# terra-render/Terra

Hardware: AMD Instinct MI355X
Metric: Msamples/s (higher is better)
Workload: dtype f32; 1 GPU; cornell_1080p_512spp; scene=cornell32, width=1920, height=1080, spp=512, bounces=8, integrator=simple, triangles=32, tree=auto, traversal=reference tree + leaf-box cull, tile=64, sample_split=8, parallelism=single

## Files before the change

include/terra_amd.h:

```cpp
#ifndef TERRA_AMD_H
#define TERRA_AMD_H

#include "Terra.h"

#ifdef __cplusplus
extern "C" {
#endif

typedef enum {
    kTerraAmdOk               = 0,
    kTerraAmdErrNoDevice      = -1,
    kTerraAmdErrNotCommitted  = -2,
    kTerraAmdErrUnsupported   = -3,
    kTerraAmdErrBadArgument   = -4,
    kTerraAmdErrLaunch        = -5
} TerraAmdStatus;

const char* terra_amd_last_error ( void );
void        terra_amd_clear_error ( void );
int         terra_amd_first_error ( char* buf, size_t capacity );
void        terra_amd_clear_first_error ( void );
size_t      terra_amd_thread_staging_bytes ( void );

int  terra_amd_init ( void );
// ... 65 lines not shown
int  terra_amd_set_job_order ( HTerraScene scene, int on );
int  terra_amd_get_job_order ( HTerraScene scene );

int  terra_amd_set_empty_skip ( HTerraScene scene, int on );
int  terra_amd_get_empty_skip ( HTerraScene scene );
int  terra_amd_empty_skip_info ( HTerraScene scene, uint32_t out[2] );
int  terra_amd_empty_proof ( const float* cam_rot9, const float* cam_pos3, float tan_half_fov, float aspect, float jitter, uint32_t fb_w, uint32_t fb_h,
                             uint32_t x0, uint32_t y0, uint32_t x1, uint32_t y1, const float* tris9, size_t n_tris );

int  terra_amd_set_leaf_box_test ( HTerraScene scene, int on );
int  terra_amd_get_leaf_box_test ( HTerraScene scene );
int  terra_amd_leaf_box_info ( HTerraScene scene, uint32_t out[2] );
int  terra_amd_set_leaf_pairs ( HTerraScene scene, int on );
int  terra_amd_get_leaf_pairs ( HTerraScene scene );
int  terra_amd_leaf_pair_info ( HTerraScene scene, uint32_t out[2] );

int  terra_amd_set_environment_lighting ( HTerraScene scene, int on );
int  terra_amd_get_environment_lighting ( HTerraScene scene );

int  terra_amd_set_sampler_integration ( HTerraScene scene, int on );
int  terra_amd_get_sampler_integration ( HTerraScene scene );

int  terra_amd_set_environment_sampling ( HTerraScene scene, int on );
int  terra_amd_get_environment_sampling ( HTerraScene scene );

int  terra_amd_set_environment_mis ( HTerraScene scene, int on );
int  terra_amd_get_environment_mis ( HTerraScene scene );

int terra_amd_set_work_counters ( HTerraScene scene, int on );
int terra_amd_get_work_counters ( HTerraScene scene );
// ... 296 lines not shown
```

terra_amd/csrc/dev_types.h:

```cpp
#pragma once
#include <stdint.h>
#include <stddef.h>
#include <hip/hip_vector_types.h>

#define TERRA_DEV_MAX_ATTR 8

struct DevF3 { float x, y, z; };
struct DevF4 { float x, y, z, w; };

#define DEV_CHILD_LEAF  0x80000000u
#define DEV_CHILD_EMPTY 0xFFFFFFFFu

struct DevNode {
    float    min0[3], max0[3];
    float    min1[3], max1[3];
    uint32_t child[2];
    uint32_t prim[2];
};
static_assert ( sizeof ( DevNode ) == 64, "DevNode must be 64 bytes" );

struct DevFastNode {
    uint32_t q[3][2][4];
    uint32_t child[4];
    uint32_t pad[4];
// ... 68 lines not shown
struct DevLeafPair { uint32_t tri[2]; uint32_t rank[2]; };
static_assert ( sizeof ( DevLeafPair ) == 16, "DevLeafPair must be 16 bytes" );
constexpr uint32_t terra_leaf_pair_words_entry_of ( uint32_t n_tris ) { return 2u * n_tris; }
constexpr uint32_t terra_leaf_pair_words_masks ( uint32_t n_tris ) { return 3u * n_tris; }
#define TERRA_PAIR_ENTRY_BYTES 64
#define TERRA_PAIR_BOX_STRIDE 48
constexpr uint32_t terra_pair_entry_offset ( uint32_t n_pairs, uint32_t perm, uint32_t e ) { return TERRA_PAIR_ENTRY_BYTES * ( perm * n_pairs + e ); }
constexpr uint32_t terra_pair_boxes_offset ( uint32_t n_pairs ) { return 6u * TERRA_PAIR_ENTRY_BYTES * n_pairs; }
constexpr uint32_t terra_pair_box_plane_offset ( uint32_t k, uint32_t a, uint32_t s ) { return TERRA_PAIR_BOX_STRIDE * k + 8u * ( 2u * a + s ); }
constexpr uint32_t terra_pair_section_bytes ( uint32_t n_pairs ) { return terra_pair_boxes_offset ( n_pairs ) + TERRA_PAIR_BOX_STRIDE * n_pairs; }
static_assert ( terra_pair_box_plane_offset ( 7, 0, 0 ) == 336 && terra_pair_box_plane_offset ( 0, 2, 1 ) + 8u == TERRA_PAIR_BOX_STRIDE, "a box = six 8-byte plane pairs; a group of eight within 384 bytes" );
#define TERRA_SHADE_CONSTS_BYTES 48u
static_assert ( terra_pair_section_bytes ( TERRA_LEAF_RANK_MAX / 2 ) + TERRA_SHADE_CONSTS_BYTES * TERRA_LEAF_RANK_MAX <= 6u * TERRA_RANKED_ENTRY_BYTES * TERRA_LEAF_RANK_MAX
                && terra_pair_section_bytes ( 1 ) + TERRA_SHADE_CONSTS_BYTES * 2u <= 6u * TERRA_RANKED_ENTRY_BYTES * 2u, "pair section + shading constants fit where the plan budgeted ranked entries" );
static_assert ( terra_pair_section_bytes ( TERRA_LEAF_RANK_MAX / 2 ) <= 6u * TERRA_RANKED_ENTRY_BYTES * TERRA_LEAF_RANK_MAX && terra_pair_section_bytes ( 1 ) <= 6u * TERRA_RANKED_ENTRY_BYTES * 2u, "the pair section never takes more LDS than the ranked entries it replaces" );
constexpr uint32_t terra_pair_key ( uint32_t rank, uint32_t tri ) { return ( rank + 1u ) << 5 | tri; }
static_assert ( TERRA_LEAF_RANK_MAX <= 32, "a pair key keeps the triangle in five bits" );
#define TERRA_LEAF_CAP_MAX 16
#define TERRA_COL 256
#define TERRA_LDS_NODE_BYTES 112
#define TERRA_AUX_WORDS 6
#define TERRA_AUX_WORDS_LDS 9
#ifndef TERRA_FAST_STACK_LDS
#define TERRA_FAST_STACK_LDS 16
#endif
#ifndef TERRA_LDS_CU_KB
#define TERRA_LDS_CU_KB 158
#endif
#ifndef TERRA_LEAF_CAP_MIN
#define TERRA_LEAF_CAP_MIN 6
// ... 119 lines not shown
```

terra_amd/csrc/render_kernels.hip:

```cpp
#include <hip/hip_runtime.h>
#include "trace_device.h"
#include "kernels.h"
#include "launch_plan.h"
#include "empty_proof.h"

#ifdef TERRA_TU
#define TERRA_TU_HAS(k) ( TERRA_TU == ( k ) )
#define TERRA_TU_MODE(k) ( TERRA_TU == ( k ) || TERRA_TU == ( k ) + 4 || TERRA_TU == ( k ) + 8 || TERRA_TU == ( k ) + 12 )
#else
#define TERRA_TU_HAS(k) ( !TERRA_RAY_SOURCE )
#define TERRA_TU_MODE(k) 1
#endif
#if TERRA_RAY_SOURCE == 3
typedef DevPointRenderParams RenderKernelParams;
#elif TERRA_RAY_SOURCE == 2
typedef DevLensRenderParams RenderKernelParams;
#elif TERRA_RAY_SOURCE == 1
typedef DevRayRenderParams RenderKernelParams;
#else
typedef DevRenderParams RenderKernelParams;
#endif

struct DevResult { float acc[3]; int samples; };

// ... 1 lines not shown
    const uint32_t v[6] = { c.rays, c.nodes, c.tri_tests, c.hits, c.rand_calls, c.attr_fetches };
    const int slot[6] = { kCtrRays, kCtrNodes, kCtrTriTests, kCtrHits, kCtrRandCalls, kCtrAttrFetches };
    #pragma unroll
    for ( int k = 0; k < 6; ++k ) {
        unsigned long long x = v[k];
        #pragma unroll
        for ( int off = 32; off > 0; off >>= 1 ) x += __shfl_xor ( x, off, 64 );
        if ( ( threadIdx.x & 63 ) == 0 && x ) atomicAdd ( &g[slot[k]], x );
    }
}

#ifndef TERRA_CHECK_SHRINK
#define TERRA_CHECK_SHRINK 0
#endif
TD const uint32_t* terra_leaf_pair_table ( const DevRenderParams& p ) {
    return p.leaf_pairs ? reinterpret_cast<const uint32_t*> ( reinterpret_cast<const char*> ( p.scene.tris ) + p.leaf_pairs ) : nullptr;
}
template <int MODE>
TD Tracer make_tracer ( const DevScene& sc, float4* lds, uint32_t stack_depth, uint32_t leaf_cap, uint32_t lds_nodes, uint32_t lds_tris, bool cull, bool fused, bool ranked,
                        const DevLeafBox* leaf_boxes, uint32_t n_leaf_boxes, const uint32_t* leaf_pairs ) {
    const int tid = threadIdx.x;
    Tracer T;
    T.sc = sc;
    float4* ln = lds;
    float4* lt = ln + ( TERRA_LDS_NODE_BYTES / 16 ) * lds_nodes;
    float4* lp = lt + 3 * lds_tris;
    uint32_t* lm = reinterpret_cast<uint32_t*> ( lp + 4 * lds_tris );
    const uint32_t m_words = MODE == 1 ? ( ( sc.n_objects * ( uint32_t ) ( sizeof ( DevMaterial ) / 4 ) + 3u ) & ~3u ) : 0u, l_words = MODE == 1 ? sc.n_lights * 4u : 0u, a_words = MODE == 1 ? ( ( sc.n_tris + 3u ) & ~3u ) : 0u;
    uint32_t* ll = lm + m_words; uint32_t* la = ll + l_words;
    ranked = MODE == 1 && ranked;
    float4* lr = reinterpret_cast<float4*> ( la + a_words );
// ... 382 lines not shown
        if ( point_inactive ( r.o, r.d ) ) j.s = p.chunk_spp;
        if ( TERRA_POINT_HOLD ) held = r;
#else
        if ( ray_record_inactive ( r ) ) j.s = p.chunk_spp;
        if ( TERRA_RAY_HOLD ) held = r;
#endif
    }
}
#endif

template <int INTEGRATOR, int COUNT, int MODE, int KINDS>
__global__ __launch_bounds__ ( 256, terra_waves ( INTEGRATOR, KINDS, MODE ) ) void terra_render_kernel ( RenderKernelParams p ) {
    extern __shared__ float4 lds_f4[];
    const int tid = threadIdx.x;
    Tracer T0 = make_tracer<MODE> ( p.scene, lds_f4, p.stack_depth, p.leaf_cap, p.lds_nodes, p.lds_tris, p.leaf_cull != 0, p.fused_slab != 0, p.leaf_rank != 0, p.leaf_boxes, p.n_leaf_boxes, terra_leaf_pair_table ( p ) );
    T0.faults = p.counters + kCtrFaults;
    if ( MODE >= 2 && p.stack_spill ) { T0.spill = p.stack_spill + ( size_t ) ( blockIdx.x * 256u + threadIdx.x ) * p.spill_cap; T0.spill_cap = p.spill_cap; }
    const Tracer T = T0;

    PixelStreams rs = trng_pixel_streams ( 0, 0, 0 );
    Counters c = counters_zero();
    float* acc_lds = reinterpret_cast<float*> ( T.stack - tid ) + ( p.stack_depth + p.leaf_cap ) * TERRA_COL + tid;
    uint32_t job_total = p.job_blocks * 256u;
    if constexpr ( MODE == 1 ) { if ( p.job_live ) job_total = *p.job_live; }
    job_init_lane ( p, acc_lds );
    Jobs jb; jb.px = jb.py = 0; jb.s = p.chunk_spp; jb.exhausted = false; jb.base = 0;
    SamplerPair sp = sampler_pair_none();
    V3 Lo = v3 ( 0, 0, 0 ), throughput = v3 ( 1, 1, 1 );
    Ray ray = make_ray ( v3 ( 0, 0, 0 ), v3 ( 0, 0, 1 ) );
    uint32_t bounce = 0;
// ... 539 lines not shown
```

terra_amd/csrc/scene_host.cpp:

```cpp
#include <hip/hip_runtime.h>
#include <algorithm>
#include <cfloat>
#include <cmath>
#include <cstdarg>
#include <cstdio>
#include <cstdlib>
#include <cstring>
#include <mutex>
#include <string>
#include <unordered_set>
#include <atomic>
#include <chrono>
#include <vector>

#include "../../include/terra_amd.h"
#include "../../include/TerraPresets.h"
#include "dev_types.h"
#include "kernels.h"
#include "launch_plan.h"
#include "empty_proof.h"
#include "tree_build.h"
#include "multi_gpu.h"

static thread_local std::string g_last_error;
// ... 287 lines not shown
    std::atomic<int> last_call { 0 };
    uint32_t sample_split = 1;
    bool env_lighting = false;
    bool work_counters = false;
    bool env_sampling = false;
    bool env_mis = false;
    int job_order = 1;
    int empty_skip = 1;
    std::atomic<uint32_t> skip_last_blocks { 0 }; std::atomic<int> skip_last_device { -1 };
    int leaf_box_test = 1;
    std::vector<DevLeafBox> leaf_boxes;
    std::atomic<uint32_t> flat_last { 0 };
    int leaf_pair_form = 1;
    std::vector<uint32_t> leaf_pairs;
    std::atomic<uint32_t> pairs_last { 0 };
    bool sampler_integration = false;
    std::string commit_error;
    std::atomic<bool> warned_camera { false };
    int test_pad_stack = 0;
    int test_fast_stack_lds = 0;
    float test_shrink_reference_boxes = 0.f;
};

static Scene* S ( HTerraScene h ) { return ( Scene* ) h; }
static const Scene::Replica& primary ( const Scene* s ) { static const Scene::Replica none; return s->replicas.empty() ? none : s->replicas[0]; }
static std::vector<int> devices_of ( const Scene* s ) { std::vector<int> d; for ( const Scene::Replica& r : s->replicas ) d.push_back ( r.device ); return d; }

static std::atomic<bool> g_commit_timing { false };
static bool timing_on() { return g_commit_timing.load ( std::memory_order_relaxed ); }
bool terra_commit_timing_on() { return timing_on(); }
// ... 117 lines not shown
extern "C" int terra_amd_set_empty_skip ( HTerraScene h, int on ) {
    if ( on < 0 || on > 1 ) return fail ( kTerraAmdErrBadArgument, "terra_amd_set_empty_skip: 0 (off) or 1 (on)" );
    S ( h )->empty_skip = on; return 0;
}
extern "C" int terra_amd_get_empty_skip ( HTerraScene h ) { return S ( h )->empty_skip; }
extern "C" int terra_amd_set_leaf_box_test ( HTerraScene h, int on ) {
    if ( on < 0 || on > 1 ) return fail ( kTerraAmdErrBadArgument, "terra_amd_set_leaf_box_test: 0 (off) or 1 (on)" );
    S ( h )->leaf_box_test = on; return 0;
}
extern "C" int terra_amd_get_leaf_box_test ( HTerraScene h ) { return S ( h )->leaf_box_test; }
extern "C" int terra_amd_set_leaf_pairs ( HTerraScene h, int on ) {
    if ( on < 0 || on > 1 ) return fail ( kTerraAmdErrBadArgument, "terra_amd_set_leaf_pairs: 0 (off) or 1 (on)" );
    S ( h )->leaf_pair_form = on; return 0;
}
extern "C" int terra_amd_get_leaf_pairs ( HTerraScene h ) { return S ( h )->leaf_pair_form; }
extern "C" int terra_amd_empty_proof ( const float* cam_rot9, const float* cam_pos3, float tan_half_fov, float aspect, float jitter, uint32_t fb_w, uint32_t fb_h,
                                       uint32_t x0, uint32_t y0, uint32_t x1, uint32_t y1, const float* tris9, size_t n_tris ) {
    if ( !cam_rot9 || !cam_pos3 || ( n_tris && !tris9 ) ) return 0;
    const TerraEmptyPlanes planes = terra_empty_planes ( cam_rot9, cam_pos3, tan_half_fov, aspect, jitter, fb_w, fb_h, x0, y0, x1, y1 );
    if ( !planes.ok ) return 0;
    for ( size_t t = 0; t < n_tris; ++t ) if ( !terra_empty_separates ( planes, tris9 + 9 * t, tris9 + 9 * t + 3, tris9 + 9 * t + 6 ) ) return 0;
    return 1;
}
extern "C" int terra_amd_set_sampler_integration ( HTerraScene h, int on ) { S ( h )->sampler_integration = on != 0; return 0; }
extern "C" int terra_amd_get_sampler_integration ( HTerraScene h ) { return S ( h )->sampler_integration ? 1 : 0; }
extern "C" void terra_amd_set_frame_seed ( HTerraScene h, uint64_t seed ) { S ( h )->frame_seed = seed; }
extern "C" uint64_t terra_amd_get_frame_seed ( HTerraScene h ) { return S ( h )->frame_seed; }

static void release_device ( Scene* s ) {
    for ( Scene::Replica& r : s->replicas ) {
// ... 160 lines not shown
    }
    if ( pairs.size() * 2 != ntri ) return none;
    std::vector<uint32_t> order ( pairs.size() );
    for ( size_t e = 0; e < order.size(); ++e ) order[e] = ( uint32_t ) e;
    auto low = [&] ( uint32_t e ) { return std::min ( pairs[e].rank[0], pairs[e].rank[1] ); };
    std::sort ( order.begin(), order.end(), [&] ( uint32_t x, uint32_t y ) { return low ( x ) < low ( y ); } );
    std::vector<uint32_t> t ( terra_leaf_pair_words_masks ( ( uint32_t ) ntri ) + boxes.size(), 0u );
    for ( size_t e = 0; e < order.size(); ++e ) {
        const DevLeafPair& p = pairs[order[e]];
        memcpy ( &t[4 * e], &p, sizeof p );
        t[terra_leaf_pair_words_entry_of ( ( uint32_t ) ntri ) + p.tri[0]] = ( uint32_t ) e; t[terra_leaf_pair_words_entry_of ( ( uint32_t ) ntri ) + p.tri[1]] = ( uint32_t ) e;
        t[terra_leaf_pair_words_masks ( ( uint32_t ) ntri ) + box_of_pair[order[e]]] |= 1u << e;
    }
    return t;
}

struct ReachTables { std::vector<DevReplay> replay; std::vector<uint32_t> leaf_parent, leaf_mask; uint64_t levels = 0, replayed = 0; };
static void build_reach_tables ( const std::vector<DevNode>& nodes, const std::vector<DevTri>& tris, const std::vector<uint32_t>& soup_of_fast, float margin, ReachTables& out ) {
    const size_t nn = nodes.size(), nt = soup_of_fast.size();
    out.replay.assign ( nn ? nn : 1, DevReplay{} );
    std::vector<uint32_t> leaf_parent_of_soup ( tris.size(), 0u );
    for ( size_t k = 0; k < nn; ++k ) for ( int c = 0; c < 2; ++c ) {
        const uint32_t w = nodes[k].child[c];
        if ( w == DEV_CHILD_EMPTY ) continue;
        if ( w & DEV_CHILD_LEAF ) { leaf_parent_of_soup[w & 0x7fffffffu] = ( uint32_t ) k; continue; }
        DevReplay& r = out.replay[w];
        memcpy ( r.bmin, c ? nodes[k].min1 : nodes[k].min0, 12 ); memcpy ( r.bmax, c ? nodes[k].max1 : nodes[k].max0, 12 );
        r.parent = ( uint32_t ) k; r.pad = 0;
    }
    auto contains = [&] ( const DevReplay & outer, const DevReplay & inner ) {
// ... 450 lines not shown
    s->tree = choose_tree ( s, f.ntri );
    TreeChoice& c = s->tree;
    if ( c.reach_cull ) for ( DevNode& d : f.nodes ) for ( int k = 0; k < 2; ++k ) {
        if ( d.child[k] == DEV_CHILD_EMPTY || ! ( d.child[k] & DEV_CHILD_LEAF ) ) continue;
        const DevTri& t = f.tris[d.child[k] & 0x7fffffffu];
        float* mn = k ? d.min1 : d.min0; float* mx = k ? d.max1 : d.max0;
        for ( int a = 0; a < 3; ++a ) {
            const float lo = std::min ( t.a[a], std::min ( t.b[a], t.c[a] ) ) - c.reach_margin, hi = std::max ( t.a[a], std::max ( t.b[a], t.c[a] ) ) + c.reach_margin;
            mn[a] = std::min ( mn[a], lo ); mx[a] = std::max ( mx[a], hi );
        }
    }
    f.leaf_boxes = leaf_box_table ( f.nodes, f.tris, f.ntri );
    s->leaf_boxes = f.leaf_boxes;
    f.leaf_pairs = leaf_pair_table ( f.leaf_boxes, f.tris, f.ntri );
    s->leaf_pairs = f.leaf_pairs;
    FastTree ft;
    if ( c.use_fast && !c.fast_on_device ) { if ( int rc = build_fast_tree_host ( s, c, f, ft ) ) return rc; }
    if ( s->tree_mode == 2 && !c.use_fast && !c.resident && f.ntri >= 2 )
        fprintf ( stderr, "[terra_amd] warning: this scene (%zu triangles) is traversed through the reference tree%s, typically 10-20 x slower than the fast tree -- %s\n", f.ntri,
                  c.cull_ok ? " with the leaf-box cull" : " decision by decision", c.note.c_str() );
    release_device ( s );
    if ( terra_amd_device_count() <= 0 ) return fail ( kTerraAmdErrNoDevice, "no HIP device visible: terra_scene_commit built the host tree but cannot upload; terra_render will fail" );
    return upload ( s, device, f, ft );
}

extern "C" void terra_scene_commit ( HTerraScene h ) {
    Scene* s = S ( h );
    const bool rebuild = s->dirty_objects || s->opts.accelerator != s->new_opts.accelerator || s->nodes.empty();
    const bool env_changed = s->env_lighting && memcmp ( &s->opts.environment_map, &s->new_opts.environment_map, sizeof ( TerraAttribute ) ) != 0;
    s->opts = s->new_opts;
// ... 214 lines not shown
    const TreeChoice& c = s->tree;
    const bool cam_ok = ray_origins_ok ? *ray_origins_ok : ( c.reach || c.reach_cull ) ? ( fabsf ( p.cam_pos[0] ) <= c.reach_limit && fabsf ( p.cam_pos[1] ) <= c.reach_limit && fabsf ( p.cam_pos[2] ) <= c.reach_limit ) : coords_within_margin ( p.cam_pos, 3 );
    if ( c.use_fast && r.dev.fast_nodes_h && ( s->tree_mode == 1 || cam_ok ) ) terra_plan_fast_tree ( p );
    else if ( ( c.use_fast || c.cull_ok ) && !cam_ok && !ray_origins_ok && !s->warned_camera.exchange ( true ) )
        fprintf ( stderr, "[terra_amd] warning: camera at (%g, %g, %g) lies outside the range (+-%g) for which this scene's traversal shortcut is proven: this call runs the reference "
                  "tree's replica traversal (same image, typically 10-20 x slower on large scenes); terra_amd_traversal_info() reports camera_limit and last_call\n",
                  ( double ) p.cam_pos[0], ( double ) p.cam_pos[1], ( double ) p.cam_pos[2], ( double ) shortcut_limit ( c ) );
    apply_stack_hooks ( s, p );
    p.leaf_cull = ( c.cull_ok && cam_ok && p.lds_mode != 2 ) ? 1u : 0u;
    p.fused_slab = ( p.leaf_cull && !c.reach_cull ) ? 1u : 0u;
    if ( s->leaf_box_test && r.d_blob && terra_leaf_boxes_fit ( p, ( uint32_t ) s->leaf_boxes.size() ) ) {
        p.leaf_boxes = ( const DevLeafBox* ) ( ( const char* ) r.d_blob + s->blob.sec[kSecLeafBoxes].offset ); p.n_leaf_boxes = ( uint32_t ) s->leaf_boxes.size();
    }
    p.leaf_pairs = 0;
    if ( s->leaf_pair_form && r.d_blob && !s->leaf_pairs.empty() && p.lds_mode == 1 && p.leaf_rank ) p.leaf_pairs = ( uint32_t ) ( s->blob.sec[kSecLeafPairs].offset - s->blob.sec[kSecTris].offset );
    if ( p.lds_mode != 1 ) p.scene.sincos24 = nullptr;
    s->last_call.store ( p.lds_mode == 2 ? ( r.dev.reach ? kTerraAmdCallFastTreeReach : kTerraAmdCallFastTree ) : ( p.leaf_cull ? kTerraAmdCallLeafCull : kTerraAmdCallReplica ), std::memory_order_relaxed );
    p.bsdf_kinds = s->bsdf_kinds;
    p.sampler_mode = 0; p.sampler_strata = ( uint32_t ) s->opts.strata;
    if ( s->sampler_integration && s->opts.sampling_method == kTerraSamplingMethodHalton ) p.sampler_mode = 1;
    if ( s->sampler_integration && s->opts.sampling_method == kTerraSamplingMethodStratified && s->opts.strata > 0 ) p.sampler_mode = 2;
    if ( p.sampler_mode ) p.bsdf_kinds |= TERRA_KIND_SAMPLER;
    if ( r.dev.env_nx && ( p.integrator == kTerraIntegratorDirect || p.integrator == kTerraIntegratorDirectMis ) ) p.bsdf_kinds |= TERRA_KIND_SAMPLER;
    else { p.scene.env_nx = 0; p.scene.env_ny = 0; }
    if ( s->env_mis && p.scene.env_nx && p.scene.env_monotone && p.integrator == kTerraIntegratorDirectMis ) p.bsdf_kinds |= TERRA_KIND_ENV_MIS;
    p.count_level = s->work_counters ? 2 : 0;
    return 0;
}

static uint64_t shard_pixels ( const DevRenderParams& p ) {
// ... 1289 lines not shown
```

terra_amd/csrc/traverse_ref.h:

```cpp
#pragma once
#include "trace_geometry.h"
#include <stddef.h>

#ifndef TERRA_PHASE_STATS
#define TERRA_PHASE_STATS 0
#endif
struct Counters {
    uint32_t rays, nodes, tri_tests, hits, rand_calls, attr_fetches;
    uint32_t tri_culled;
#if TERRA_PHASE_STATS
    uint32_t ps[16];
#endif
};
TD Counters counters_zero() {
    Counters c; c.rays = c.nodes = c.tri_tests = c.hits = c.rand_calls = c.attr_fetches = c.tri_culled = 0;
#if TERRA_PHASE_STATS
    for ( int i = 0; i < 16; ++i ) c.ps[i] = 0;
#endif
    return c;
}
#if TERRA_PHASE_STATS
#define PS_WAVE(c, k) do { if ( ( int ) ( threadIdx.x & 63 ) == __ffsll ( ( long long ) __ballot ( 1 ) ) - 1 ) ++( c ).ps[k]; } while ( 0 )
#define PS_LANE(c, k) do { ++( c ).ps[k]; } while ( 0 )
#else
// ... 17 lines not shown
    const float4* l_consts = nullptr;
    uint32_t      n_boxes;
    uint32_t      lds_nodes, lds_tris;
    int*          stack;
    int*          leaves;
    int           leaf_cap;
    int           stack_cap;
    uint32_t      stack_lim;
    uint32_t*     spill;
    uint32_t      spill_cap;
    unsigned long long* faults;
    bool cull;
    bool fused;
    bool ranked;
    bool pairs;
};
TD Tracer unstaged_tracer ( const DevScene& sc, int* words, uint32_t stack_depth, uint32_t leaf_cap, uint32_t* spill, uint32_t spill_cap ) {
    Tracer T;
    T.sc = sc; T.l_nodes = nullptr; T.l_tris = nullptr; T.l_props = nullptr; T.l_ranked = nullptr; T.n_boxes = 0;
    T.l_mats = sc.mats; T.l_lights = sc.lights; T.l_area = sc.tri_area;
    T.lds_nodes = 0; T.lds_tris = 0; T.ranked = false; T.pairs = false;
    T.stack = words + threadIdx.x; T.leaves = words + stack_depth * TERRA_COL + threadIdx.x; T.leaf_cap = ( int ) leaf_cap; T.stack_cap = ( int ) stack_depth;
    T.stack_lim = ( uint32_t ) ( uintptr_t ) words + stack_depth * 1024u;
    T.spill = spill ? spill + ( size_t ) ( blockIdx.x * 256u + threadIdx.x ) * spill_cap : nullptr; T.spill_cap = spill ? spill_cap : 0u;
    T.faults = nullptr; T.cull = false; T.fused = false;
    return T;
}

struct Closest { float depth; uint32_t tri; };

// ... 67 lines not shown

template <int COUNT, int MODE, bool ANYHIT = false>
TD void leaf_step ( const Tracer& T, const int* entry, const RayState& st, V3 o_perm, Closest& best, Counters& c, uint32_t expected = 0xffffffffu, bool* stop = nullptr ) {
    const float4* g_tris = reinterpret_cast<const float4*> ( T.sc.tris );
    PS_WAVE ( c, kPsLeafIter ); PS_LANE ( c, kPsLeafLanes );
    const uint32_t ti = ( uint32_t ) * entry;
    if ( ti == ( DEV_CHILD_EMPTY & 0x7fffffffu ) ) return;
    const TriPerm tp = MODE == 1 ? tri_perm_lds ( T.l_tris + 12 * ti, st ) : tri_perm ( g_tris[3 * ti], g_tris[3 * ti + 1], g_tris[3 * ti + 2], st );
    if ( COUNT ) ++c.tri_tests;
    float depth;
    if ( watertight_permuted ( tp, o_perm, st, depth ) && depth < best.depth ) { best.depth = depth; best.tri = ti; if ( ANYHIT && ti != expected ) *stop = true; }
}

typedef float PlanePair __attribute__ (( ext_vector_type ( 2 ) ));
typedef const __attribute__ (( address_space ( 3 ) )) PlanePair* LdsPlanes;
TD void leaf_box_test ( uint32_t bx, uint32_t by, uint32_t bz, const char* pm, const Ray& r, const SlabSel& sel, uint32_t& leaf_set, Counters& c ) {
    PS_WAVE ( c, kPsNodeIter ); PS_LANE ( c, kPsNodeLanes );
    const PlanePair ax = * ( LdsPlanes ) ( uintptr_t ) bx, ay = * ( LdsPlanes ) ( uintptr_t ) by, az = * ( LdsPlanes ) ( uintptr_t ) bz;
    const uint32_t m = *reinterpret_cast<const uint32_t*> ( pm );
    float te;
    const bool hit = slab_near_far_fused ( ax.x, ax.y, ay.x, ay.y, az.x, az.y, r, sel.oi, te );
    leaf_set |= hit ? m : 0u;
}
template <int N, uint32_t STRIDE>
TD void leaf_box_group ( uint32_t& bx, uint32_t& by, uint32_t& bz, const char*& pm, const Ray& r, const SlabSel& sel, uint32_t& leaf_set, Counters& c ) {
    #pragma unroll
    for ( int k = 0; k < N; ++k )
        leaf_box_test ( bx + STRIDE * k, by + STRIDE * k, bz + STRIDE * k, pm + TERRA_LEAF_BOX_MASK_STRIDE * k, r, sel, leaf_set, c );
    bx += STRIDE * N; by += STRIDE * N; bz += STRIDE * N; pm += TERRA_LEAF_BOX_MASK_STRIDE * N;
}
template <bool PAIRS>
TD uint32_t leaf_boxes_flat ( const Tracer& T, const Ray& r, const SlabSel& sel, Counters& c ) {
    constexpr uint32_t kStride = PAIRS ? ( uint32_t ) TERRA_PAIR_BOX_STRIDE : ( uint32_t ) TERRA_LEAF_BOX_STRIDE;
    constexpr uint32_t kX = PAIRS ? terra_pair_box_plane_offset ( 0, 0, 0 ) : terra_leaf_box_plane_offset ( 0, 0, 0 ), kY = PAIRS ? terra_pair_box_plane_offset ( 0, 1, 0 ) : terra_leaf_box_plane_offset ( 0, 1, 0 ),
                       kZ = PAIRS ? terra_pair_box_plane_offset ( 0, 2, 0 ) : terra_leaf_box_plane_offset ( 0, 2, 0 );
    const uint32_t table = ( uint32_t ) ( uintptr_t ) T.l_ranked + ( PAIRS ? terra_pair_boxes_offset ( T.lds_tris >> 1 ) : 0u );
    constexpr uint32_t kNeg = PAIRS ? terra_pair_box_plane_offset ( 0, 0, 1 ) - terra_pair_box_plane_offset ( 0, 0, 0 ) : terra_leaf_box_plane_offset ( 0, 0, 1 ) - terra_leaf_box_plane_offset ( 0, 0, 0 );
    uint32_t sx = r.inv.x < 0.f ? kNeg : 0u, sy = r.inv.y < 0.f ? kNeg : 0u, sz = r.inv.z < 0.f ? kNeg : 0u;
    asm ( "" : "+v" ( sx ), "+v" ( sy ), "+v" ( sz ) );
    uint32_t bx = table + kX + sx, by = table + kY + sy, bz = table + kZ + sz;
    asm ( "" : "+v" ( bx ), "+v" ( by ), "+v" ( bz ) );
    const char* pm = reinterpret_cast<const char*> ( T.l_props ) + terra_leaf_box_mask_offset ( 0 );
    uint32_t leaf_set = 0u;
    #pragma clang loop vectorize(disable) interleave(disable) unroll(disable)
    for ( uint32_t g = T.n_boxes / TERRA_LEAF_BOX_GROUP; g != 0; --g ) leaf_box_group<TERRA_LEAF_BOX_GROUP, kStride> ( bx, by, bz, pm, r, sel, leaf_set, c );
    if ( T.n_boxes & 4u ) leaf_box_group<4, kStride> ( bx, by, bz, pm, r, sel, leaf_set, c );
    #pragma clang loop vectorize(disable) interleave(disable) unroll(disable)
    for ( uint32_t k = T.n_boxes % 4u; k != 0; --k ) leaf_box_group<1, kStride> ( bx, by, bz, pm, r, sel, leaf_set, c );
    return leaf_set;
}

template <int COUNT, int MODE, bool FAST, bool FUSED, bool ANYHIT>
TD void traverse_pairs ( const Tracer& T, const Ray& r, const RayState& st, V3 o_perm, Closest& best, Counters& c ) {
    const SlabSel sel = slab_sel ( r );
    uint32_t leaf_set = 0u;
    PS_WAVE ( c, kPsDrainIter );
    bool flat = false;
    if constexpr ( FUSED ) flat = T.n_boxes != 0u;
    if ( flat ) leaf_set = leaf_boxes_flat<true> ( T, r, sel, c );
    else {
        int* sp = T.stack; int* lp = nullptr;
        *sp = 0; sp += TERRA_COL;
        while ( sp != T.stack ) node_step<COUNT, MODE, FAST, FUSED, true> ( T, r, sel, sp, lp, leaf_set, c );
    }
    const uint32_t perm = 2u * ( uint32_t ) st.iz + ( uint32_t ) ( st.ix != ( st.iz == 2 ? 0 : st.iz + 1 ) );
    const float4* copy = T.l_ranked + ( TERRA_PAIR_ENTRY_BYTES / 16 ) * ( T.lds_tris >> 1 ) * perm;
    float depth_best = best.depth; uint32_t key_best = ANYHIT ? best.tri : 0u;
    bool beaten = false;
    while ( leaf_set != 0u ) {
        PS_WAVE ( c, kPsLeafIter ); PS_LANE ( c, kPsLeafLanes );
        const float4* e = copy + ( TERRA_PAIR_ENTRY_BYTES / 16 ) * ( uint32_t ) __builtin_ctz ( leaf_set );
        leaf_set &= leaf_set - 1u;
        const uint2 keys = *reinterpret_cast<const uint2*> ( e + 3 );
        auto load = [&] ( bool again ) {
            uint32_t a = ( uint32_t ) ( uintptr_t ) e;
            if ( again ) asm volatile ( "" : "+v" ( a ) );
            typedef float Piece __attribute__ (( ext_vector_type ( 4 ) ));
            const __attribute__ (( address_space ( 3 ) )) Piece* q = ( const __attribute__ (( address_space ( 3 ) )) Piece* ) ( uintptr_t ) a;
            const Piece q0 = q[0], q1 = q[1], q2 = q[2];
            return PairPerm { { q0.x, q0.y, q0.z }, { q0.w, q1.x, q1.y }, { q1.z, q1.w, q2.x }, { q2.y, q2.z, q2.w } };
        };
        watertight_pair ( load, o_perm, st, [&] ( float depth, bool second ) {
            const uint32_t key = second ? keys.y : keys.x;
            if ( ( depth < depth_best ) | ( ( depth == depth_best ) & ( key < key_best ) ) ) {
                if ( ANYHIT ) { beaten = true; leaf_set = 0u; }
                else { depth_best = depth; key_best = key; }
            }
        } );
    }
    best.depth = depth_best;
    best.tri = ANYHIT ? ( beaten ? 0u : key_best ) : ( key_best ? ( key_best & 31u ) : 0xffffffffu );
}

template <int COUNT, int MODE, bool FAST, bool FUSED = false, bool ANYHIT = false>
TD void traverse_ranked ( const Tracer& T, const Ray& r, const RayState& st, V3 o_perm, Closest& best, Counters& c, uint32_t expected ) {
    if constexpr ( COUNT == 0 ) if ( T.pairs ) { traverse_pairs<COUNT, MODE, FAST, FUSED, ANYHIT> ( T, r, st, o_perm, best, c ); return; }
    const SlabSel sel = slab_sel ( r );
    uint32_t leaf_set = 0u;
    PS_WAVE ( c, kPsDrainIter );
    bool flat = false;
    if constexpr ( COUNT == 0 && FUSED ) flat = T.n_boxes != 0u;
    if ( flat ) leaf_set = leaf_boxes_flat<false> ( T, r, sel, c );
    else {
        int* sp = T.stack; int* lp = nullptr;
        *sp = 0; sp += TERRA_COL;
        while ( sp != T.stack ) node_step<COUNT, MODE, FAST, FUSED, true> ( T, r, sel, sp, lp, leaf_set, c );
    }
    const uint32_t perm = 2u * ( uint32_t ) st.iz + ( uint32_t ) ( st.ix != ( st.iz == 2 ? 0 : st.iz + 1 ) );
    const float4* copy = T.l_ranked + 3u * T.lds_tris * perm;
    while ( leaf_set != 0u ) {
        PS_WAVE ( c, kPsLeafIter ); PS_LANE ( c, kPsLeafLanes );
        const float4* e = copy + 3u * ( uint32_t ) __builtin_ctz ( leaf_set );
        leaf_set &= leaf_set - 1u;
        const float4 q0 = e[0], q1 = e[1], q2 = e[2];
        const TriPerm tp = { { q0.x, q0.y, q0.z }, { q0.w, q1.x, q1.y }, { q1.z, q1.w, q2.x } };
        if ( COUNT ) ++c.tri_tests;
        float depth;
// ... 59 lines not shown
```

terra_amd/runtime.py:

```python
from __future__ import annotations

import ctypes as C
from pathlib import Path
from typing import Optional, Tuple

import numpy as np

from . import api, scenes

HERE = Path(__file__).resolve().parent
import os as _os
LIB_PATH = Path(_os.environ.get("TERRA_AMD_LIB", HERE / "libterra_amd.so"))

_lib: Optional[api.TerraLib] = None


class TerraAmdError(RuntimeError):
    pass


class Stats(C.Structure):
    _fields_ = [(n, C.c_uint64) for n in ("rays", "nodes", "box_tests", "tri_tests", "hits", "samples", "rand_calls", "attr_fetches", "pixels", "launches", "tri_culled")]

    def as_dict(self):
# ... 54 lines not shown
    "terra_amd_traversal_info": (C.c_int, [C.c_void_p, C.POINTER(TraversalInfo)]),
    "terra_amd_set_tree_builder": (C.c_int, [C.c_void_p, C.c_int]),
    "terra_amd_get_tree_builder": (C.c_int, [C.c_void_p]),
    "terra_amd_set_job_order": (C.c_int, [C.c_void_p, C.c_int]),
    "terra_amd_get_job_order": (C.c_int, [C.c_void_p]),
    "terra_amd_set_empty_skip": (C.c_int, [C.c_void_p, C.c_int]),
    "terra_amd_get_empty_skip": (C.c_int, [C.c_void_p]),
    "terra_amd_empty_skip_info": (C.c_int, [C.c_void_p, C.POINTER(C.c_uint32)]),
    "terra_amd_set_leaf_box_test": (C.c_int, [C.c_void_p, C.c_int]),
    "terra_amd_get_leaf_box_test": (C.c_int, [C.c_void_p]),
    "terra_amd_leaf_box_info": (C.c_int, [C.c_void_p, C.POINTER(C.c_uint32)]),
    "terra_amd_scene_leaf_boxes": (C.c_int, [C.c_void_p, C.c_void_p, C.c_int]),
    "terra_amd_set_leaf_pairs": (C.c_int, [C.c_void_p, C.c_int]),
    "terra_amd_get_leaf_pairs": (C.c_int, [C.c_void_p]),
    "terra_amd_leaf_pair_info": (C.c_int, [C.c_void_p, C.POINTER(C.c_uint32)]),
    "terra_amd_scene_leaf_pairs": (C.c_int, [C.c_void_p, C.c_void_p, C.c_int]),
    "terra_amd_scene_leaf_pair_masks": (C.c_int, [C.c_void_p, C.c_void_p, C.c_int]),
    "terra_amd_leaf_pair_offsets": (C.c_int, [C.c_uint32, C.c_void_p, C.c_void_p]),
    "terra_amd_empty_proof": (C.c_int, [C.c_void_p, C.c_void_p, C.c_float, C.c_float, C.c_float] + [C.c_uint32] * 6 + [C.c_void_p, C.c_size_t]),
    "terra_amd_set_sample_split": (C.c_int, [C.c_void_p, C.c_int]),
    "terra_amd_get_sample_split": (C.c_int, [C.c_void_p]),
    "terra_amd_auto_sample_split": (C.c_int, [C.c_size_t, C.c_size_t, C.c_size_t, C.c_int, C.c_size_t, C.c_int]),
    "terra_amd_set_environment_lighting": (C.c_int, [C.c_void_p, C.c_int]),
    "terra_amd_get_environment_lighting": (C.c_int, [C.c_void_p]),
    "terra_amd_get_stats": (C.c_int, [C.c_void_p, C.POINTER(Stats)]),
    "terra_amd_reset_stats": (C.c_int, [C.c_void_p]),
    "terra_amd_scene_info": (C.c_int, [C.c_void_p, C.POINTER(SceneInfo)]),
    "terra_amd_scene_bvh_nodes": (C.c_int, [C.c_void_p, C.c_void_p, C.c_int]),
    "terra_amd_scene_leaf_ranks": (C.c_int, [C.c_void_p, C.c_void_p, C.c_int]),
    "terra_amd_render_device": (C.c_int, [_CAM, C.c_void_p, C.c_void_p, C.c_void_p] + [_SZ] * 6 + [C.c_void_p, C.c_void_p]),
# ... 490 lines not shown
```

Before: 33560 Msamples/s.

## Visit nearest leaf pair box first and cut farther boxes early

During the flat leaf-box test each hit box's entry depth is packed with its index into a sortable key, and the two nearest boxes are tracked. When every pair has its own box, the drain loop visits the nearest box first and stops once the best hit is closer than the second box's entry, with an early exit for any-hit rays. The aim is fewer triangle pair intersection tests per ray, at the cost of extra min/max work per box test and a flag bit packed into the pair-table offset.

```diff
diff --git a/include/terra_amd.h b/include/terra_amd.h
--- a/include/terra_amd.h
+++ b/include/terra_amd.h
@@ -103,6 +103,8 @@
 int  terra_amd_set_leaf_pairs ( HTerraScene scene, int on );
 int  terra_amd_get_leaf_pairs ( HTerraScene scene );
 int  terra_amd_leaf_pair_info ( HTerraScene scene, uint32_t out[2] );
+int  terra_amd_set_leaf_nearest_first ( HTerraScene scene, int on );
+int  terra_amd_get_leaf_nearest_first ( HTerraScene scene );
 
 int  terra_amd_set_environment_lighting ( HTerraScene scene, int on );
 int  terra_amd_get_environment_lighting ( HTerraScene scene );
diff --git a/terra_amd/csrc/dev_types.h b/terra_amd/csrc/dev_types.h
--- a/terra_amd/csrc/dev_types.h
+++ b/terra_amd/csrc/dev_types.h
@@ -106,6 +106,7 @@
 static_assert ( terra_pair_section_bytes ( TERRA_LEAF_RANK_MAX / 2 ) + TERRA_SHADE_CONSTS_BYTES * TERRA_LEAF_RANK_MAX <= 6u * TERRA_RANKED_ENTRY_BYTES * TERRA_LEAF_RANK_MAX
                 && terra_pair_section_bytes ( 1 ) + TERRA_SHADE_CONSTS_BYTES * 2u <= 6u * TERRA_RANKED_ENTRY_BYTES * 2u, "pair section + shading constants fit where the plan budgeted ranked entries" );
 static_assert ( terra_pair_section_bytes ( TERRA_LEAF_RANK_MAX / 2 ) <= 6u * TERRA_RANKED_ENTRY_BYTES * TERRA_LEAF_RANK_MAX && terra_pair_section_bytes ( 1 ) <= 6u * TERRA_RANKED_ENTRY_BYTES * 2u, "the pair section never takes more LDS than the ranked entries it replaces" );
+#define TERRA_LEAF_PAIRS_NEAREST 1u
 constexpr uint32_t terra_pair_key ( uint32_t rank, uint32_t tri ) { return ( rank + 1u ) << 5 | tri; }
 static_assert ( TERRA_LEAF_RANK_MAX <= 32, "a pair key keeps the triangle in five bits" );
 #define TERRA_LEAF_CAP_MAX 16
diff --git a/terra_amd/csrc/render_kernels.hip b/terra_amd/csrc/render_kernels.hip
--- a/terra_amd/csrc/render_kernels.hip
+++ b/terra_amd/csrc/render_kernels.hip
@@ -39,7 +39,7 @@
 #define TERRA_CHECK_SHRINK 0
 #endif
 TD const uint32_t* terra_leaf_pair_table ( const DevRenderParams& p ) {
-    return p.leaf_pairs ? reinterpret_cast<const uint32_t*> ( reinterpret_cast<const char*> ( p.scene.tris ) + p.leaf_pairs ) : nullptr;
+    return p.leaf_pairs ? reinterpret_cast<const uint32_t*> ( reinterpret_cast<const char*> ( p.scene.tris ) + ( p.leaf_pairs & ~TERRA_LEAF_PAIRS_NEAREST ) ) : nullptr;
 }
 template <int MODE>
 TD Tracer make_tracer ( const DevScene& sc, float4* lds, uint32_t stack_depth, uint32_t leaf_cap, uint32_t lds_nodes, uint32_t lds_tris, bool cull, bool fused, bool ranked,
@@ -452,6 +452,7 @@
     extern __shared__ float4 lds_f4[];
     const int tid = threadIdx.x;
     Tracer T0 = make_tracer<MODE> ( p.scene, lds_f4, p.stack_depth, p.leaf_cap, p.lds_nodes, p.lds_tris, p.leaf_cull != 0, p.fused_slab != 0, p.leaf_rank != 0, p.leaf_boxes, p.n_leaf_boxes, terra_leaf_pair_table ( p ) );
+    if constexpr ( MODE == 1 && COUNT == 0 ) T0.nearest = T0.pairs && T0.n_boxes != 0u && ( p.leaf_pairs & TERRA_LEAF_PAIRS_NEAREST ) != 0u;
     T0.faults = p.counters + kCtrFaults;
     if ( MODE >= 2 && p.stack_spill ) { T0.spill = p.stack_spill + ( size_t ) ( blockIdx.x * 256u + threadIdx.x ) * p.spill_cap; T0.spill_cap = p.spill_cap; }
     const Tracer T = T0;
diff --git a/terra_amd/csrc/scene_host.cpp b/terra_amd/csrc/scene_host.cpp
--- a/terra_amd/csrc/scene_host.cpp
+++ b/terra_amd/csrc/scene_host.cpp
@@ -325,6 +325,8 @@
     int leaf_pair_form = 1;
     std::vector<uint32_t> leaf_pairs;
     std::atomic<uint32_t> pairs_last { 0 };
+    int leaf_nearest_first = 1;
+    bool pair_per_box = false;
     bool sampler_integration = false;
     std::string commit_error;
     std::atomic<bool> warned_camera { false };
@@ -472,6 +474,11 @@
     S ( h )->leaf_pair_form = on; return 0;
 }
 extern "C" int terra_amd_get_leaf_pairs ( HTerraScene h ) { return S ( h )->leaf_pair_form; }
+extern "C" int terra_amd_set_leaf_nearest_first ( HTerraScene h, int on ) {
+    if ( on < 0 || on > 1 ) return fail ( kTerraAmdErrBadArgument, "terra_amd_set_leaf_nearest_first: 0 (off) or 1 (on)" );
+    S ( h )->leaf_nearest_first = on; return 0;
+}
+extern "C" int terra_amd_get_leaf_nearest_first ( HTerraScene h ) { return S ( h )->leaf_nearest_first; }
 extern "C" int terra_amd_empty_proof ( const float* cam_rot9, const float* cam_pos3, float tan_half_fov, float aspect, float jitter, uint32_t fb_w, uint32_t fb_h,
                                        uint32_t x0, uint32_t y0, uint32_t x1, uint32_t y1, const float* tris9, size_t n_tris ) {
     if ( !cam_rot9 || !cam_pos3 || ( n_tris && !tris9 ) ) return 0;
@@ -662,6 +669,11 @@
     }
     return t;
 }
+static bool leaf_pairs_one_per_box ( const std::vector<uint32_t>& table, size_t n_boxes, size_t ntri ) {
+    if ( table.empty() || n_boxes * 2 != ntri ) return false;
+    for ( size_t k = 0; k < n_boxes; ++k ) if ( table[terra_leaf_pair_words_masks ( ( uint32_t ) ntri ) + k] != 1u << k ) return false;
+    return true;
+}
 
 struct ReachTables { std::vector<DevReplay> replay; std::vector<uint32_t> leaf_parent, leaf_mask; uint64_t levels = 0, replayed = 0; };
 static void build_reach_tables ( const std::vector<DevNode>& nodes, const std::vector<DevTri>& tris, const std::vector<uint32_t>& soup_of_fast, float margin, ReachTables& out ) {
@@ -1142,6 +1154,7 @@
     s->leaf_boxes = f.leaf_boxes;
     f.leaf_pairs = leaf_pair_table ( f.leaf_boxes, f.tris, f.ntri );
     s->leaf_pairs = f.leaf_pairs;
+    s->pair_per_box = leaf_pairs_one_per_box ( f.leaf_pairs, f.leaf_boxes.size(), f.ntri );
     FastTree ft;
     if ( c.use_fast && !c.fast_on_device ) { if ( int rc = build_fast_tree_host ( s, c, f, ft ) ) return rc; }
     if ( s->tree_mode == 2 && !c.use_fast && !c.resident && f.ntri >= 2 )
@@ -1386,6 +1399,7 @@
     }
     p.leaf_pairs = 0;
     if ( s->leaf_pair_form && r.d_blob && !s->leaf_pairs.empty() && p.lds_mode == 1 && p.leaf_rank ) p.leaf_pairs = ( uint32_t ) ( s->blob.sec[kSecLeafPairs].offset - s->blob.sec[kSecTris].offset );
+    if ( p.leaf_pairs && ! ( p.leaf_pairs & 3u ) && p.n_leaf_boxes && s->leaf_nearest_first && s->pair_per_box ) p.leaf_pairs |= TERRA_LEAF_PAIRS_NEAREST;
     if ( p.lds_mode != 1 ) p.scene.sincos24 = nullptr;
     s->last_call.store ( p.lds_mode == 2 ? ( r.dev.reach ? kTerraAmdCallFastTreeReach : kTerraAmdCallFastTree ) : ( p.leaf_cull ? kTerraAmdCallLeafCull : kTerraAmdCallReplica ), std::memory_order_relaxed );
     p.bsdf_kinds = s->bsdf_kinds;
diff --git a/terra_amd/csrc/traverse_ref.h b/terra_amd/csrc/traverse_ref.h
--- a/terra_amd/csrc/traverse_ref.h
+++ b/terra_amd/csrc/traverse_ref.h
@@ -55,6 +55,7 @@
     bool fused;
     bool ranked;
     bool pairs;
+    bool nearest = false;
 };
 TD Tracer unstaged_tracer ( const DevScene& sc, int* words, uint32_t stack_depth, uint32_t leaf_cap, uint32_t* spill, uint32_t spill_cap ) {
     Tracer T;
@@ -152,23 +153,35 @@
 
 typedef float PlanePair __attribute__ (( ext_vector_type ( 2 ) ));
 typedef const __attribute__ (( address_space ( 3 ) )) PlanePair* LdsPlanes;
-TD void leaf_box_test ( uint32_t bx, uint32_t by, uint32_t bz, const char* pm, const Ray& r, const SlabSel& sel, uint32_t& leaf_set, Counters& c ) {
+#define TERRA_NO_BOX 0x7fffffff
+struct NearestBoxes { int32_t lo, hi; };
+template <bool PAIRS>
+TD void leaf_box_test ( uint32_t bx, uint32_t by, uint32_t bz, const char* pm, const Ray& r, const SlabSel& sel, uint32_t& leaf_set, Counters& c, uint32_t entry, NearestBoxes& nb ) {
     PS_WAVE ( c, kPsNodeIter ); PS_LANE ( c, kPsNodeLanes );
     const PlanePair ax = * ( LdsPlanes ) ( uintptr_t ) bx, ay = * ( LdsPlanes ) ( uintptr_t ) by, az = * ( LdsPlanes ) ( uintptr_t ) bz;
     const uint32_t m = *reinterpret_cast<const uint32_t*> ( pm );
     float te;
     const bool hit = slab_near_far_fused ( ax.x, ax.y, ay.x, ay.y, az.x, az.y, r, sel.oi, te );
     leaf_set |= hit ? m : 0u;
-}
-template <int N, uint32_t STRIDE>
-TD void leaf_box_group ( uint32_t& bx, uint32_t& by, uint32_t& bz, const char*& pm, const Ray& r, const SlabSel& sel, uint32_t& leaf_set, Counters& c ) {
+    if constexpr ( PAIRS ) {
+        uint32_t bits;
+        asm ( "v_bfi_b32 %0, 31, %1, %2" : "=v" ( bits ) : "s" ( entry ), "v" ( te ) );
+        const int32_t key = hit ? ( int32_t ) bits : TERRA_NO_BOX;
+        const int32_t lo = nb.lo, hi = nb.hi;
+        nb.lo = key < lo ? key : lo;
+        nb.hi = __builtin_elementwise_max ( __builtin_elementwise_min ( lo, hi ), __builtin_elementwise_min ( __builtin_elementwise_max ( lo, hi ), key ) );
+    }
+}
+template <int N, uint32_t STRIDE, bool PAIRS>
+TD void leaf_box_group ( uint32_t& bx, uint32_t& by, uint32_t& bz, const char*& pm, const Ray& r, const SlabSel& sel, uint32_t& leaf_set, Counters& c, uint32_t& entry, NearestBoxes& nb ) {
     #pragma unroll
     for ( int k = 0; k < N; ++k )
-        leaf_box_test ( bx + STRIDE * k, by + STRIDE * k, bz + STRIDE * k, pm + TERRA_LEAF_BOX_MASK_STRIDE * k, r, sel, leaf_set, c );
+        leaf_box_test<PAIRS> ( bx + STRIDE * k, by + STRIDE * k, bz + STRIDE * k, pm + TERRA_LEAF_BOX_MASK_STRIDE * k, r, sel, leaf_set, c, entry + ( uint32_t ) k, nb );
     bx += STRIDE * N; by += STRIDE * N; bz += STRIDE * N; pm += TERRA_LEAF_BOX_MASK_STRIDE * N;
+    if constexpr ( PAIRS ) entry += ( uint32_t ) N;
 }
 template <bool PAIRS>
-TD uint32_t leaf_boxes_flat ( const Tracer& T, const Ray& r, const SlabSel& sel, Counters& c ) {
+TD uint32_t leaf_boxes_flat ( const Tracer& T, const Ray& r, const SlabSel& sel, Counters& c, NearestBoxes& nb ) {
     constexpr uint32_t kStride = PAIRS ? ( uint32_t ) TERRA_PAIR_BOX_STRIDE : ( uint32_t ) TERRA_LEAF_BOX_STRIDE;
     constexpr uint32_t kX = PAIRS ? terra_pair_box_plane_offset ( 0, 0, 0 ) : terra_leaf_box_plane_offset ( 0, 0, 0 ), kY = PAIRS ? terra_pair_box_plane_offset ( 0, 1, 0 ) : terra_leaf_box_plane_offset ( 0, 1, 0 ),
                        kZ = PAIRS ? terra_pair_box_plane_offset ( 0, 2, 0 ) : terra_leaf_box_plane_offset ( 0, 2, 0 );
@@ -179,12 +192,13 @@
     uint32_t bx = table + kX + sx, by = table + kY + sy, bz = table + kZ + sz;
     asm ( "" : "+v" ( bx ), "+v" ( by ), "+v" ( bz ) );
     const char* pm = reinterpret_cast<const char*> ( T.l_props ) + terra_leaf_box_mask_offset ( 0 );
-    uint32_t leaf_set = 0u;
+    uint32_t leaf_set = 0u, entry = 0u;
+    if constexpr ( PAIRS ) nb.lo = nb.hi = TERRA_NO_BOX;
     #pragma clang loop vectorize(disable) interleave(disable) unroll(disable)
-    for ( uint32_t g = T.n_boxes / TERRA_LEAF_BOX_GROUP; g != 0; --g ) leaf_box_group<TERRA_LEAF_BOX_GROUP, kStride> ( bx, by, bz, pm, r, sel, leaf_set, c );
-    if ( T.n_boxes & 4u ) leaf_box_group<4, kStride> ( bx, by, bz, pm, r, sel, leaf_set, c );
+    for ( uint32_t g = T.n_boxes / TERRA_LEAF_BOX_GROUP; g != 0; --g ) leaf_box_group<TERRA_LEAF_BOX_GROUP, kStride, PAIRS> ( bx, by, bz, pm, r, sel, leaf_set, c, entry, nb );
+    if ( T.n_boxes & 4u ) leaf_box_group<4, kStride, PAIRS> ( bx, by, bz, pm, r, sel, leaf_set, c, entry, nb );
     #pragma clang loop vectorize(disable) interleave(disable) unroll(disable)
-    for ( uint32_t k = T.n_boxes % 4u; k != 0; --k ) leaf_box_group<1, kStride> ( bx, by, bz, pm, r, sel, leaf_set, c );
+    for ( uint32_t k = T.n_boxes % 4u; k != 0; --k ) leaf_box_group<1, kStride, PAIRS> ( bx, by, bz, pm, r, sel, leaf_set, c, entry, nb );
     return leaf_set;
 }
 
@@ -195,7 +209,9 @@
     PS_WAVE ( c, kPsDrainIter );
     bool flat = false;
     if constexpr ( FUSED ) flat = T.n_boxes != 0u;
-    if ( flat ) leaf_set = leaf_boxes_flat<true> ( T, r, sel, c );
+    NearestBoxes nb; nb.lo = nb.hi = TERRA_NO_BOX;
+    bool nearest = false;
+    if ( flat ) { leaf_set = leaf_boxes_flat<true> ( T, r, sel, c, nb ); nearest = T.nearest; }
     else {
         int* sp = T.stack; int* lp = nullptr;
         *sp = 0; sp += TERRA_COL;
@@ -205,10 +221,13 @@
     const float4* copy = T.l_ranked + ( TERRA_PAIR_ENTRY_BYTES / 16 ) * ( T.lds_tris >> 1 ) * perm;
     float depth_best = best.depth; uint32_t key_best = ANYHIT ? best.tri : 0u;
     bool beaten = false;
+    const float cut = __uint_as_float ( ( uint32_t ) ( nearest ? nb.hi : TERRA_NO_BOX ) & ~31u );
+    if ( ANYHIT && nearest && depth_best < __uint_as_float ( ( uint32_t ) nb.lo & ~31u ) ) leaf_set = 0u;
+    uint32_t next = nearest ? ( uint32_t ) nb.lo & 31u : ( uint32_t ) __builtin_ctz ( leaf_set | 0x80000000u );
     while ( leaf_set != 0u ) {
         PS_WAVE ( c, kPsLeafIter ); PS_LANE ( c, kPsLeafLanes );
-        const float4* e = copy + ( TERRA_PAIR_ENTRY_BYTES / 16 ) * ( uint32_t ) __builtin_ctz ( leaf_set );
-        leaf_set &= leaf_set - 1u;
+        const float4* e = copy + ( TERRA_PAIR_ENTRY_BYTES / 16 ) * next;
+        leaf_set &= ~ ( 1u << next );
         const uint2 keys = *reinterpret_cast<const uint2*> ( e + 3 );
         auto load = [&] ( bool again ) {
             uint32_t a = ( uint32_t ) ( uintptr_t ) e;
@@ -225,6 +244,8 @@
                 else { depth_best = depth; key_best = key; }
             }
         } );
+        if ( depth_best < cut ) leaf_set = 0u;
+        next = ( uint32_t ) __builtin_ctz ( leaf_set | 0x80000000u );
     }
     best.depth = depth_best;
     best.tri = ANYHIT ? ( beaten ? 0u : key_best ) : ( key_best ? ( key_best & 31u ) : 0xffffffffu );
@@ -238,7 +259,8 @@
     PS_WAVE ( c, kPsDrainIter );
     bool flat = false;
     if constexpr ( COUNT == 0 && FUSED ) flat = T.n_boxes != 0u;
-    if ( flat ) leaf_set = leaf_boxes_flat<false> ( T, r, sel, c );
+    NearestBoxes no_nb;
+    if ( flat ) leaf_set = leaf_boxes_flat<false> ( T, r, sel, c, no_nb );
     else {
         int* sp = T.stack; int* lp = nullptr;
         *sp = 0; sp += TERRA_COL;
diff --git a/terra_amd/runtime.py b/terra_amd/runtime.py
--- a/terra_amd/runtime.py
+++ b/terra_amd/runtime.py
@@ -92,6 +92,8 @@
     "terra_amd_set_leaf_pairs": (C.c_int, [C.c_void_p, C.c_int]),
     "terra_amd_get_leaf_pairs": (C.c_int, [C.c_void_p]),
     "terra_amd_leaf_pair_info": (C.c_int, [C.c_void_p, C.POINTER(C.c_uint32)]),
+    "terra_amd_set_leaf_nearest_first": (C.c_int, [C.c_void_p, C.c_int]),
+    "terra_amd_get_leaf_nearest_first": (C.c_int, [C.c_void_p]),
     "terra_amd_scene_leaf_pairs": (C.c_int, [C.c_void_p, C.c_void_p, C.c_int]),
     "terra_amd_scene_leaf_pair_masks": (C.c_int, [C.c_void_p, C.c_void_p, C.c_int]),
     "terra_amd_leaf_pair_offsets": (C.c_int, [C.c_uint32, C.c_void_p, C.c_void_p]),
```

After: 36350 Msamples/s (median of 6 runs). 1.08x the previous value.
